# jan-frost/uzliti_slam

Hardware: AMD Instinct MI355X
Metric: SE(3) edges optimized/sec (node-pairs matched/sec in `secondary`) (higher is better)
Workload: dtype f64; 1 GPU; BASELINE config 2: 1000-node / 5000-edge SE(3) pose graph, 20 LM iterations, Huber(1) on loop closures; one independent graph per GPU; system_edges=4999

## Files before the change

uzliti_slam_amd/csrc/pgo_handle.hpp:

```cpp
#pragma once
#include "uzl_common.hpp"
#include "pgo_types.hpp"
#include "pgo_schur.hpp"
#include "pgo_ml_plan.hpp"
#include "pgo_lm.hpp"

#include <algorithm>
#include <chrono>
#include <cstdlib>
#include <cmath>
#include <functional>
#include <limits>
#include <new>
#include <numeric>

namespace uzl {
void k_prepare_nodes(const uzl_node* nodes, int n, int xy, double* pose, hipStream_t s);
void k_prepare_flat_nodes(const double* poses12, int n, double* pose, hipStream_t s);
void k_prepare_edges(const uzl_edge* edges, const int32_t* src, int e, const double* sensors, int ns, int xy, int odom_params,
                     double* zinv, double* info, hipStream_t s);
void k_prepare_flat_edges(const double* meas12, const double* info36, int e, double* zinv, double* info, hipStream_t s);
int k_chi2(const PgoDev& D, const double* pose, double delta, hipStream_t s);
int k_chi2_trial(const PgoDev& D, const double* pose, double delta, hipStream_t s);
hipError_t k_hessian(const PgoDev& D, const double* pose, double delta, int* g_edges, int* g_rows, hipStream_t s, bool with_chi2 = true, hipEvent_t ev_a = nullptr,
// ... 20 lines not shown
void k_poses_out(const double* pose, int n, double* out12, hipStream_t s);
void k_schur_gather(const PgoDev& D, const SchurDev& S, hipStream_t s);
void k_lm_head(const LmSlot* slots, int nslots, int pass_flags, hipStream_t s);
void k_lm_tail(const LmSlot* slots, int nslots, hipStream_t s);
hipError_t kl_linearize(const LmSlot* sl, int nslots, int g_edges, int g_asm, hipStream_t s);
void kl_eval(const LmSlot* sl, int nslots, int g_edges, int g_oplus, hipStream_t s);
void kl_schur_reduce(const LmSlot* sl, const LmShape& sh, hipStream_t s);
void kl_schur_backsub(const LmSlot* sl, const LmShape& sh, hipStream_t s);
void kl_schur_reduce(const HostSlot& hs, const LmShape& sh, hipStream_t s, KernelTimer* timer);
void kl_schur_backsub(const HostSlot& hs, const LmShape& sh, hipStream_t s, KernelTimer* timer);
void kl_ml_numeric(const LmSlot* sl, const LmShape& sh, int which, hipStream_t s);
void kl_ml_trial(const LmSlot* sl, const LmShape& sh, int which, int ns_steps, hipStream_t s);
void kl_ml_numeric(const HostSlot& hs, const LmShape& sh, hipStream_t s, KernelTimer* timer, const std::function<void()>& level1_done);
void kl_ml_trial(const HostSlot& hs, const LmShape& sh, int ns_steps, hipStream_t s, KernelTimer* timer);
void ml_cg_variant(const MlHot& ml, int agg, size_t lds_full, int32_t* variant, int32_t* comp_u, uint64_t* lds);
hipError_t kl_ml_init(const LmSlot* sl, const LmSlot* by_value, const LmShape& sh, hipStream_t s);
hipError_t kl_ml_pcg_its(const LmSlot* sl, const LmSlot* by_value, const LmShape& sh, int first, int n, hipStream_t s, hipEvent_t* ev = nullptr);
void kl_ml_pcg_init(const HostSlot& hs, const LmShape& sh, hipStream_t s);
void kl_ml_spmv(const HostSlot& hs, const LmShape& sh, int parity, hipStream_t s, hipEvent_t ev_a = nullptr, hipEvent_t ev_b = nullptr);
hipError_t kl_ml_cg(const HostSlot& hs, const LmShape& sh, int parity, int init, hipStream_t s, hipEvent_t ev_a = nullptr, hipEvent_t ev_b = nullptr);
}



namespace uzl { struct LmRun; }
using namespace uzl;

struct SysBufs {
    DevBuf<int32_t> row_ptr, col, rowhdr, b2v;
    DevBuf<double> blk, hdiag, minv, x, xs, r, z, p, p2, ap;
    std::vector<int32_t> upload(int nb, const std::vector<int32_t>& h_row_ptr, const std::vector<int32_t>& h_col, const std::vector<int32_t>& h_b2v, hipStream_t s)
    {
// ... 157 lines not shown
```

uzliti_slam_amd/csrc/pgo_lm.hpp:

```cpp
#pragma once
#include <cmath>
#include <hip/hip_runtime.h>

#include "pgo_types.hpp"

namespace uzl {

#define UZL_HD __host__ __device__ __forceinline__

constexpr double kResidualGuard = 0.25;
constexpr double kRateDrop = 0.6;
constexpr double kTolFloor2 = 1e-4;
constexpr double kStepT = 1.0, kStepR = 0.1;

UZL_HD double lm_cube(double t)
{
#pragma clang fp contract(off)
    const double p = t * t, pe = fma(t, t, -p);
    const double q = p * t, qe = fma(p, t, -q);
    return q + (qe + pe * t);
}

UZL_HD double lm_log(double x)
{
// ... 17 lines not shown
UZL_HD double lm_pcg_rate(double rz_stop, double rz_end, int its, double tol2, double tol_f2)
{
#pragma clang fp contract(off)
    const double rz0 = rz_stop / (tol2 * tol_f2);
    return (its >= 16 && rz0 > 0. && rz_end > 0. && rz_end < rz0) ? lm_log(rz0 / rz_end) / its : -1.;
}

UZL_HD bool lm_refresh(int it, int iterations, bool may_run_last, double last_rel, double refresh_rel, double rate_ref, double rate_last,
                       double rate_drop = kRateDrop)
{
#pragma clang fp contract(off)
    return it == 0 || ((last_rel > refresh_rel || (rate_ref > 0. && rate_last > 0. && rate_last < rate_drop * rate_ref)) &&
                       (may_run_last || it + 1 < iterations));
}

struct LmStep { double rho; bool accepted; double last_rel; };
UZL_HD LmStep lm_step(double current_chi, double temp_chi, double scale_sum, double& lambda, double& ni)
{
#pragma clang fp contract(off)
    LmStep r;
    const double scale = scale_sum + 1e-3;
    r.rho = (current_chi - temp_chi) / scale;
    r.accepted = r.rho > 0 && std::isfinite(temp_chi);
    r.last_rel = 0.;
    if (r.accepted) {
        double alpha = 1. - lm_cube(2 * r.rho - 1);
        alpha = alpha < 2. / 3. ? alpha : 2. / 3.;
        const double scaleFactor = (1. / 3. > alpha) ? 1. / 3. : alpha;
        lambda *= scaleFactor;
        ni = 2.;
// ... 11 lines not shown
```

uzliti_slam_amd/csrc/pgo_lm_kernels.hip:

```cpp
#include "pgo_device.hpp"
#include "pgo_lm.hpp"

namespace uzl {

__device__ __forceinline__ void lm_head_decide(const LmSlot& S, LmDev* lm, int phase, double chi, double dmax, int pass_flags)
{
    const int p = lm->pass + 1;
    lm->pass = p;
    double* __restrict__ scal = S.D.scal;
    int need = 0;
    if (phase == kLmLin) {
        scal[4] = chi; scal[6] = dmax;
        if (lm->it == 0) {
            lm->chi_cur = chi; lm->chi2_initial = chi;
            lm->lambda = 1e-5 * dmax;
            lm->ni = 2.;
        }
        lm->adopted = 0;
        if (lm->pending) { lm->ix ^= 1; lm->pending = 0; lm->adopted = 1; }
        if (lm_refresh(lm->it, lm->iterations, lm->sync_rebuild != 0, lm->last_rel, lm->refresh_rel, lm->rate_ref, lm->rate_last, lm->rate_drop)) {
            lm->st_precond_builds++;
            need |= (lm->it == 0 || lm->sync_rebuild) ? (kNeedNumeric | kNeedTrial) : kNeedRebuild;
        }
        lm->qmax = 0;
        if (S.red) lm->schur_pass = p;
    } else if (phase == kLmRetry) {
        if (S.red) lm->schur_pass = p;
    } else if (phase == kLmNeedSetup) {
        need = lm->need;
    } else {
        return;
    }
    const double lambda = lm->lambda;
    scal[3] = lambda; scal[8] = lm->tol_f2; scal[12] = lm->eps_t; scal[13] = lm->eps_r;
// ... 88 lines not shown
        ratio = bb > 0. ? rr / bb : 0.;
    }
    __shared__ uint32_t s_seq;
    if (tid == 0) {
        const uint32_t seq = (uint32_t)(lm->tails + 1);
        lm->tails = (int32_t)seq;
        s_seq = seq;
        double* __restrict__ scal = sscal;
        if (solving && !done) {
            if (lm->flags[1] >= lm->max_it) { lm->phase = kLmAnomaly; lm->anomaly_code = 1; lm->flags[0] = 1; }
        } else if (solving) {
            const int its = lm->flags[1];
            bool conv = lm->flags[2] == 0;
            if (conv) scal[7] = ratio;
            if (conv && lm->guarded && !(ratio <= kResidualGuard)) conv = false;
            if (!conv) { lm->phase = kLmAnomaly; lm->anomaly_code = lm->flags[2] ? 2 : 3; }
            else {
                scal[4] = chi_t; scal[5] = sc;
                lm->st_pcg_iterations += its; lm->st_lm_trials++; lm->pcg_last = its;
                const double rate = lm_pcg_rate(scal[1], scal[0], its, lm->tol2, lm->tol_f2);
                if (rate > 0.) { lm->rate_last = rate; if (lm->fresh || lm->rate_ref < 0.) lm->rate_ref = rate; }
                double lambda = lm->lambda, ni = lm->ni;
                const LmStep st = lm_step(lm->chi_cur, chi_t, sc, lambda, ni);
                lm->lambda = lambda; lm->ni = ni;
                if (st.accepted) { lm->last_rel = st.last_rel; lm->chi_cur = chi_t; lm->cur ^= 1; }
                const int qmax = lm->qmax + 1;
                lm->qmax = qmax;
                if (st.rho < 0 && qmax < 10) lm->phase = kLmRetry;
                else {
                    lm->st_iterations_done = lm->it + 1;
                    if (qmax == 10 || st.rho == 0) { lm->st_terminated_early = 1; lm->phase = kLmDone; }
// ... 34 lines not shown
```

uzliti_slam_amd/csrc/pgo_ml_kernels.hip:

```cpp
#include <hip/hip_ext.h>
#include <functional>
#include <mutex>
#include <type_traits>

#include "pgo_device.hpp"
#include "uzl_common.hpp"

namespace uzl {

#ifdef UZL_STAMPS
__device__ unsigned long long g_stamps[64];
#define STAMP_DECL unsigned long long st_prev_ = __builtin_amdgcn_s_memrealtime(); int st_i_ = 0;
#define STAMP(base) do { if (blockIdx.x == 0 && threadIdx.x == 0) { unsigned long long n_ = __builtin_amdgcn_s_memrealtime(); \
        atomicAdd(&g_stamps[(base) + st_i_], n_ - st_prev_); st_prev_ = n_; } st_i_++; } while (0)
#else
#define STAMP_DECL
#define STAMP(base) do { } while (0)
#endif

struct P3 { double X[9], Y[9], Z[9]; };

__device__ __forceinline__ void mat3(const double* A, const double* B, double* C)
{
#pragma unroll
// ... 1134 lines not shown
        sr1[tid] = s;
        if (gl == 1 && A1 < n1) rg[(size_t)A1 * 6 + k] = s;
    }
    __syncthreads();
    if (gl == 2 && tid < 6) {
        double s = 0.;
        for (int la = 0; la < kAggPerBlk; la++) {
            const int A1 = blockIdx.x * kAggPerBlk + la;
            if (A1 < n1) s += restrict_comp(H.geo[1] + (size_t)A1 * 3, sr1 + la * 6, tid);
        }
        rg[(size_t)blockIdx.x * 6 + tid] = s;
    }
    if (blockIdx.x == 0 && tid == 0) { D.flags[0] = 0; D.flags[1] = 0; D.flags[2] = 0; D.flags[3] = 0; D.scal[2] = 1.; }
}

__device__ __forceinline__ double dot6(double2 a0, double2 a1, double2 a2, double v0, double v1, double v2, double v3, double v4, double v5)
{
    double t = a0.x * v0;
    t = fma(a0.y, v1, t); t = fma(a1.x, v2, t); t = fma(a1.y, v3, t); t = fma(a2.x, v4, t); t = fma(a2.y, v5, t);
    return t;
}
template <int AGG>
__device__ __forceinline__ double sg_at(const double* __restrict__ Sg, int gl, int t)
{
    if (AGG == 1 || gl != 2) return Sg[t];
    const double2 v = reinterpret_cast<const double2*>(Sg)[t];
    return v.x + v.y;
}
constexpr int kSpmvWaves4 = 4;
__device__ __forceinline__ int xcd_contiguous(int b, int g)
{
    const int q = g >> 3, rem = g & 7, x = b & 7;
    return x * q + (x < rem ? x : rem) + (b >> 3);
}
template <int AGG, int RPW = AGG, int WAVES = (AGG == 1 ? 8 : kSpmvWaves4)>
__device__ __forceinline__ void ml_spmv_kernel_body(PgoDev D, MlHot H, const double* __restrict__ p_old,
                                                     double* __restrict__ p_new, int n_part, double tol2)
{
    constexpr int kWaves = WAVES, kRowsPerWave = RPW;
    constexpr bool kLds = (WAVES == 2);
    constexpr int kRowsPerBlk = kWaves * kRowsPerWave, kAggPerBlk = kRowsPerBlk / kMlFanout;
    constexpr int kGrpU = (kWaves >= 8) ? 2 : 4;
    __shared__ double sgrp[kMaxPartials / 64];
    __shared__ double slook[2][kMaxPartials / 64];
    constexpr int kGat = 2 + 3 * kRowsPerWave;
    __shared__ __attribute__((aligned(16))) double sgat[kWaves][kGat][64];
    __shared__ double sd[kRowsPerBlk * 6];
    __shared__ double sw[kRowsPerBlk * 6];
    __shared__ double ss1[kAggPerBlk * 6];
    __shared__ double sg1[kAggPerBlk * 3];
    const int done = D.flags[0];
    STAMP_DECL
    const int gl = (AGG == 1 || H.levels < 2) ? 1 : 2;
    const int tid = threadIdx.x, lane = tid & 63, wv = __builtin_amdgcn_readfirstlane(tid >> 6), g = lane / 6, r = lane % 6;
    const bool lact = lane < 60;
    const int bx = xcd_contiguous((int)blockIdx.x, (int)gridDim.x);
    const int row0 = bx * kRowsPerBlk + wv * kRowsPerWave;
    double vpart[kGrpU];
#pragma unroll
    for (int u = 0; u < kGrpU; u++) {
        const int i = (wv + u * kWaves) * 64 + lane;
        const double x = D.part_b[i < n_part ? i : 0];
        vpart[u] = (i < n_part) ? x : 0.;
    }
    double2 vlook[kGrpU];
    if (bx == 0) {
#pragma unroll
// ... 4 lines not shown
        }
    }
    const int it = D.flags[1];
    const double rz_prev = D.scal[2], thr_old = D.scal[1], lambda = D.scal[3], rz_last = D.scal[0];
    int s0[kRowsPerWave], s1[kRowsPerWave], cf[kRowsPerWave], cf2[kRowsPerWave];
#pragma unroll
    for (int q = 0; q < kRowsPerWave; q++) {
        const int a = row0 + q;
        const int32_t* __restrict__ hd = D.rowhdr + (size_t)(a < D.nb ? a : 0) * kRowHdr;
        s0[q] = (a < D.nb) ? hd[0] : 0;
        s1[q] = (a < D.nb) ? hd[1] : 0;
        cf[q] = (a < D.nb && lact) ? hd[2 + g] : -1;
        cf2[q] = (a < D.nb && lact) ? hd[12 + g] : -1;
    }
    if (done) return;
    double g1v = 0.;
    if (tid < kAggPerBlk * 3) {
        const int A1 = bx * kAggPerBlk + tid / 3;
        if (gl == 2 && A1 < H.n[1]) g1v = H.geo[1][(size_t)A1 * 3 + tid % 3];
    }
    const int gbase = g * 6;
    auto gather6 = [&](int slot, double v, int base, double& v0, double& v1, double& v2, double& v3, double& v4, double& v5) {
        double* line = sgat[wv][slot];
        line[lane] = v;
        __builtin_amdgcn_wave_barrier();
        const double2* __restrict__ p2 = reinterpret_cast<const double2*>(line + base);
        const double2 a = p2[0], b = p2[1], c = p2[2];
        v0 = a.x; v1 = a.y; v2 = b.x; v3 = b.y; v4 = c.x; v5 = c.y;
    };
    double hrow[6] = {0, 0, 0, 0, 0, 0}, zo_r = 0., po_r = 0.;
// ... 603 lines not shown
    const int done = D.flags[0];
    const int tid = threadIdx.x, t = blockIdx.x * 256 + tid, n6 = 6 * H.n[2];
    double vp[4];
    part_issue<256, 4>(D.part_a, n_part, tid, vp);
    double rgv = 0., sgv = 0.;
    if (t < n6) { rgv = rg_old[t]; sgv = sg_at<4>(H.Sg, 2, t); }
    const double rz = D.scal[0];
    if (done) return;
    const double pAp = block_sum_w<4>(part_fold<256, 4>(D.part_a, n_part, tid, vp), s4);
    const bool bad = !(pAp > 0.);
    const double alpha = bad ? 0. : rz / pAp;
    if (t < n6) H.Vg[t] = rgv - alpha * sgv;
    if (blockIdx.x == 0 && tid == 0) { D.scal[9] = alpha; D.scal[10] = bad ? 1. : 0.; }
}

template <int kCompU, bool kLds = false>
__device__ __forceinline__ void ml_cg_comp_kernel_body(PgoDev D, MlHot H, const double* __restrict__ p,
                                                           const double* __restrict__ rg_old, double* __restrict__ rg_new,
                                                           int n_part, int init)
{
    __shared__ double s3[3];
    __shared__ double sv[kCgBlk];
    __shared__ double sw[kCgBlk];
    __shared__ double sy[6];
    __shared__ double szj[48];
    __shared__ double scomp[3][6];
    __shared__ double spm[6];
    if (D.flags[0]) return;
    const int tid = threadIdx.x;
    const int a = blockIdx.x * kMlFanout + tid / 6, r = tid % 6;
    const bool act = tid < 48 && a < D.nb;
    const int n1 = H.n[1], ng6 = 6 * n1;
    double vpart[4] = {0., 0., 0., 0.};
    if (!init) part_issue<kCgBlk, 4>(D.part_a, n_part, tid, vpart);
    double xv = 0., xsv = 0., rv0 = 0., apv = 0., pv = 0., geo[12] = {0, 0, 0, 0, 0, 0, 0, 0, 0, 0, 0, 0};
    const int look = init ? 1 : D.flags[3];
    const double unit = progress_unit(D.scal, r);
    if (act) {
        const size_t i = (size_t)a * 6 + r;
        rv0 = D.r[i];
        if (!init) { xv = D.x[i]; xsv = D.xs[i]; apv = D.ap[i]; pv = p[i]; }
        const double* __restrict__ gg = H.geo0 + (size_t)a * 12;
#pragma unroll
// ... 7 lines not shown
        for (int c = 0; c < 6; c++) { const double2 v = src[c]; w0[2 * c] = v.x; w0[2 * c + 1] = v.y; }
    }
    const double rz = init ? 0. : D.scal[0];
    double rgreg[kCompU], sgreg[kCompU];
    float cm[6][kCompU];
    const int cst = H.c32_stride;
    const float* __restrict__ crow = H.Cmat32 + (size_t)blockIdx.x * 6 * cst;
#pragma unroll
    for (int u = 0; u < kCompU; u++) {
        const int t = u * kCgBlk + tid;
        const bool in = t < ng6;
        rgreg[u] = in ? rg_old[t] : 0.;
        sgreg[u] = (!init && in) ? H.Sg[t] : 0.;
#pragma unroll
        for (int q = 0; q < 6; q++) { const float y = crow[(size_t)q * cst + (in ? t : 0)]; cm[q][u] = in ? y : 0.f; }
    }
    double alpha = 0.;
    bool bad = false;
    if (!init) {
        const double pAp = block_sum_w<3, kLds>(part_fold<kCgBlk, 4>(D.part_a, n_part, tid, vpart), s3);
        bad = !(pAp > 0.);
        alpha = bad ? 0. : rz / pAp;
    }
    {
        double ps[6] = {0, 0, 0, 0, 0, 0};
#pragma unroll
        for (int u = 0; u < kCompU; u++) {
            const double v = fma(-alpha, sgreg[u], rgreg[u]);
#pragma unroll
            for (int q = 0; q < 6; q++) ps[q] = fma((double)cm[q][u], v, ps[q]);
// ... 297 lines not shown
    const auto* lm = state_of(S, slots);
    const int ix = lm->ix;
    if (init) {
        if (!init_due(lm)) return;
        ml_cg_kernel_body<AGG, COMP, YPRE, false>(S.Dp, hot_of(S, ix), S.pbuf[0], rg_of(S, ix, 0), rg_of(S, ix, 1), 0, 1);
    } else ml_cg_kernel_body<AGG, COMP, YPRE, VPRE>(S.Dp, hot_of(S, ix), S.pbuf[parity ^ 1], rg_of(S, ix, parity ^ 1), rg_of(S, ix, parity), S.g_spmv, 0);
}
template <class SLOT>
__global__ __launch_bounds__(256) void ml_alpha_lm_kernel(const SLOT slots, int parity)
{
    const LmSlot& S = slot_of(slots);
    const auto* lm = state_of(S, slots);
    ml_alpha_kernel_body(S.Dp, hot_of(S, lm->ix), rg_of(S, lm->ix, parity ^ 1), S.g_spmv);
}

static hipError_t lm_cg_lds(const void* fn, int variant_ix, size_t lds)
{
    constexpr int kMaxDev = 16, kVar = 24;
    static size_t configured_tab[kMaxDev][kVar] = {};
    static std::mutex mu;
    int dev = 0;
    if (hipGetDevice(&dev) != hipSuccess || dev < 0 || dev >= kMaxDev) dev = 0;
    std::lock_guard<std::mutex> lock(mu);
    if (lds > configured_tab[dev][variant_ix]) {
        const hipError_t e = hipFuncSetAttribute(fn, hipFuncAttributeMaxDynamicSharedMemorySize, (int)lds);
        if (e != hipSuccess) return e;
        configured_tab[dev][variant_ix] = lds;
    }
    return hipSuccess;
}

template <class SLOT>
static hipError_t kl_ml_cg_t(SLOT sl, const LmShape& sh, int parity, int init, hipStream_t s, hipEvent_t ev_a = nullptr, hipEvent_t ev_b = nullptr)
{
    constexpr int kSlotKind = std::is_pointer<SLOT>::value ? 0 : (std::is_same<SLOT, LmSlot>::value ? 1 : 2);
    const dim3 g(sh.g_rows, 1, sh.nslots), t(kCgBlk);
    const size_t lds = (size_t)sh.cg_lds;
    if (lds > kMlLdsLimit) return hipErrorInvalidValue;
    auto cg = [&](auto kernel) {
        const hipError_t e = lm_cg_lds(reinterpret_cast<const void*>(kernel), 8 * kSlotKind + sh.cg_variant, lds);
        if (e == hipSuccess) launch(kernel, g, t, lds, s, ev_a, ev_b, sl, parity, init);
        return e;
    };
    switch (sh.cg_variant) {
    case kCgComp1: {
        const int u = sh.comp_u;
        auto kernel = sh.batch_geometry ? (u <= 5 ? ml_cg_comp_lm_kernel<5, true, SLOT> : ml_cg_comp_lm_kernel<8, true, SLOT>)
                    : u <= 5 ? ml_cg_comp_lm_kernel<5, false, SLOT> : u <= 8 ? ml_cg_comp_lm_kernel<8, false, SLOT>
                    : u <= 12 ? ml_cg_comp_lm_kernel<12, false, SLOT> : ml_cg_comp_lm_kernel<16, false, SLOT>;
        launch(kernel, g, t, 0, s, ev_a, ev_b, sl, parity, init);
        return hipSuccess; }
    case kCgPlain1: return cg(ml_cg_lm_kernel<1, false, false, false, SLOT>);
    case kCgPlain4: return cg(ml_cg_lm_kernel<4, false, false, false, SLOT>);
    case kCgComp4: return cg(ml_cg_lm_kernel<4, true, false, false, SLOT>);
    case kCgComp4Ypre: return cg(ml_cg_lm_kernel<4, true, true, false, SLOT>);
    case kCgComp4Vpre:
        if (!init) hipLaunchKernelGGL((ml_alpha_lm_kernel<SLOT>), dim3((6 * sh.n_lv[2] + 255) / 256, 1, sh.nslots), dim3(256), 0, s, sl, parity);
        return cg(ml_cg_lm_kernel<4, true, false, true, SLOT>);
    }
    return hipErrorInvalidValue;
// ... 20 lines not shown
void ml_cg_variant(const MlHot& ml, int agg, size_t lds_full, int32_t* variant, int32_t* comp_u, uint64_t* lds)
{
    *comp_u = 0; *lds = lds_full;
    if (agg == 1) {
        if (!ml.Cmat) { *variant = kCgPlain1; return; }
        const int cols = 6 * ml.n[1];
        *variant = kCgComp1; *lds = 0;
        *comp_u = cols <= 5 * kCgBlk ? 5 : (cols <= 8 * kCgBlk ? 8 : (cols <= 12 * kCgBlk ? 12 : 16));
        return;
    }
    if (!ml.Cmat) { *variant = kCgPlain4; return; }
    *lds = ml_comp4_lds(ml.n[2]);
    const bool ypre = ml.levels >= 2 && 6 * ml.n[2] <= 4 * 32 * kYU;
    *variant = ypre ? kCgComp4Ypre : (ml.Vg != nullptr ? kCgComp4Vpre : kCgComp4);
}
hipError_t kl_ml_init(const LmSlot* sl, const LmSlot* by_value, const LmShape& sh, hipStream_t s)
{
    if (by_value && sh.nslots == 1) { kl_ml_init_t<LmSlot>(*by_value, sh, s); return kl_ml_cg_t<LmSlot>(*by_value, sh, 0, 1, s); }
    kl_ml_init_t<const LmSlot*>(sl, sh, s);
    return kl_ml_cg_t<const LmSlot*>(sl, sh, 0, 1, s);
}
hipError_t kl_ml_pcg_its(const LmSlot* sl, const LmSlot* by_value, const LmShape& sh, int first, int n, hipStream_t s, hipEvent_t* ev)
{
    const bool one = by_value && sh.nslots == 1 && !ev;
    for (int q = 0; q < n; q++) {
        const int par = (first + q) & 1;
        hipError_t e;
        if (ev) { kl_ml_spmv_t<const LmSlot*>(sl, sh, par, s, ev[4 * q], ev[4 * q + 1]); e = kl_ml_cg_t<const LmSlot*>(sl, sh, par, 0, s, ev[4 * q + 2], ev[4 * q + 3]); }
        else if (one) { kl_ml_spmv_t<LmSlot>(*by_value, sh, par, s); e = kl_ml_cg_t<LmSlot>(*by_value, sh, par, 0, s); }
        else { kl_ml_spmv_t<const LmSlot*>(sl, sh, par, s); e = kl_ml_cg_t<const LmSlot*>(sl, sh, par, 0, s); }
        if (e != hipSuccess) return e;
    }
    return hipSuccess;
}
void kl_ml_pcg_init(const HostSlot& hs, const LmShape& sh, hipStream_t s) { kl_ml_init_t<HostSlot>(hs, sh, s); }
void kl_ml_spmv(const HostSlot& hs, const LmShape& sh, int parity, hipStream_t s, hipEvent_t ev_a, hipEvent_t ev_b) { kl_ml_spmv_t<HostSlot>(hs, sh, parity, s, ev_a, ev_b); }
hipError_t kl_ml_cg(const HostSlot& hs, const LmShape& sh, int parity, int init, hipStream_t s, hipEvent_t ev_a, hipEvent_t ev_b)
{
    return kl_ml_cg_t<HostSlot>(hs, sh, parity, init, s, ev_a, ev_b);
}

}

#ifdef UZL_STAMPS
extern "C" UZL_DIAG_EXPORT int uzl_debug_read_stamps(unsigned long long* out, int reset)
{
    if (hipMemcpyFromSymbol(out, HIP_SYMBOL(uzl::g_stamps), sizeof(unsigned long long) * 64) != hipSuccess) return -3;
    if (reset) { unsigned long long z[64] = {0}; if (hipMemcpyToSymbol(HIP_SYMBOL(uzl::g_stamps), z, sizeof(z)) != hipSuccess) return -3; }
    return 0;
}
#endif

#ifdef UZL_DIAG
// ... 51 lines not shown
```

uzliti_slam_amd/csrc/pgo_types.hpp:

```cpp
#pragma once
#include <cstdint>
#include "../../include/uzl_mi355x.h"

namespace uzl {
constexpr size_t kMlLdsLimit = (size_t)140 * 1024;
__host__ __device__ inline size_t ml_comp4_lds(int n2) { return (size_t)6 * (size_t)n2 * 8 + 64; }


constexpr int kMaxPartials = 8192;
constexpr int kProgressEvery = 2;
constexpr int kRowHdr = 24;

struct PgoDev {
    int32_t n, nb, e, nslots;
    int32_t e_begin, e_end;
    int32_t diag_owner;
    int32_t sibling0;
    double* pose;
    double* pose_trial;
    const int32_t* v2b;
    const int32_t* b2v;
    const int32_t* ei;
    const int32_t* ej;
    const double* zinv;
// ... 157 lines not shown
    double* rg[2][2];
    double* dense[2][kMlMaxLevels + 1];
    double* nsT[2];
    double* nsX[2];
    double* pbuf[2];
    double* pose[2];
    int32_t g_edges, g_asm, g_oplus, g_rows, g_spmv, red, pad0, pad1;
    int64_t copy_stride;
};
struct HostSlot {
    LmSlot S;
    int32_t ix, cur;
    double tol2;
};

enum LmCgVariant : int32_t { kCgPlain1 = 0, kCgComp1 = 1, kCgPlain4 = 2, kCgComp4 = 3, kCgComp4Ypre = 4, kCgComp4Vpre = 5 };
struct LmShape {
    int32_t nslots;
    int32_t batch_geometry;
    int32_t levels, cl, agg;
    int32_t mult, ns_steps, upper_ns;
    int32_t cg_variant, comp_u;
    int32_t n_lv[kMlMaxLevels + 2];
    int32_t work_t[kMlMaxLevels + 2];
    int32_t chunks[kMlMaxLevels + 2];
    int32_t inner_aggs;
    int32_t g_edges, g_asm, g_oplus, g_rows, g_spmv;
    int32_t red, schur_runs, schur_backsub_grid;
    int64_t schur_items;
    uint64_t cg_lds;
// ... 11 lines not shown
```

uzliti_slam_amd/csrc/uzl_pgo_lm.hip:

```cpp
#include "pgo_handle.hpp"

namespace uzl {

struct LmRun {
    int nslots = 0;
    DevBuf<LmSlot> d_slots;
    DevBuf<LmDev> d_lm;
    PinBuf<LmHost> h_pub;
    LmHost* d_pub = nullptr;
    PinBuf<LmDev> h_init;
    std::vector<LmSlot> slots;
    LmShape shape{};
    DevBuf<double> d_start;
    hipEvent_t ev_fork = nullptr, ev_join = nullptr;
    bool join_pending = false;
    uint64_t gen = ~0ull;
    int solves_of_gen = 0;
    int first_solve_its = 0;
    std::vector<std::vector<int>> trial_its_prev, trial_its_cur;
    std::vector<uint64_t> hist_gen;
    struct Seg { hipGraph_t g = nullptr; hipGraphExec_t x = nullptr; };
    Seg setup, reb, pcg_long;
    void drop(Seg& q) { if (q.x) { (void)hipGraphExecDestroy(q.x); q.x = nullptr; } if (q.g) { (void)hipGraphDestroy(q.g); q.g = nullptr; } }
    void drop_all() { drop(setup); drop(reb); drop(pcg_long); }
};

void lm_run_destroy(LmRun* r)
{
    if (!r) return;
    r->drop_all();
    if (r->ev_fork) (void)hipEventDestroy(r->ev_fork);
    if (r->ev_join) (void)hipEventDestroy(r->ev_join);
    delete r;
}

namespace {

LmRun* new_run()
{
// ... 20 lines not shown
    UZL_HIP(kl_linearize(R->d_slots.p, sh.nslots, sh.g_edges, sh.g_asm, s));
}
void enq_head(LmRun* R, int pass_flags, bool linearized, hipStream_t s)
{
    const LmShape& sh = R->shape;
    if (!linearized) enq_linearize(R, s);
    k_lm_head(R->d_slots.p, sh.nslots, pass_flags, s);
    if (sh.red) kl_schur_reduce(R->d_slots.p, sh, s);
}
void enq_setup(LmRun* R, int which, int ns_steps, hipStream_t s)
{
    kl_ml_numeric(R->d_slots.p, R->shape, which, s);
    kl_ml_trial(R->d_slots.p, R->shape, which, ns_steps, s);
}
const LmSlot* by_value_slot(LmRun* R) { return (R->shape.nslots == 1 && !R->shape.batch_geometry) ? R->slots.data() : nullptr; }
void enq_init(LmRun* R, hipStream_t s) { UZL_HIP(kl_ml_init(R->d_slots.p, by_value_slot(R), R->shape, s)); }
void enq_pcg(LmRun* R, int first, int n, hipStream_t s, hipEvent_t* ev = nullptr) { UZL_HIP(kl_ml_pcg_its(R->d_slots.p, by_value_slot(R), R->shape, first, n, s, ev)); }
void enq_tail(LmRun* R, hipStream_t s)
{
    const LmShape& sh = R->shape;
    if (sh.red) kl_schur_backsub(R->d_slots.p, sh, s);
    kl_eval(R->d_slots.p, sh.nslots, sh.g_edges, sh.g_oplus, s);
    k_lm_tail(R->d_slots.p, sh.nslots, s);
}
template <class F>
void run_seg(LmRun::Seg& q, bool eager, hipStream_t s, F&& enqueue)
{
    if (eager) { enqueue(s); return; }
    if (!q.x) {
        UZL_HIP(hipStreamBeginCapture(s, hipStreamCaptureModeThreadLocal));
        try { enqueue(s); }
        catch (...) {
// ... 220 lines not shown
                }
                const bool no_history = jobs[(size_t)slot_job[sl]].h->cfg.pass_history == 1;
                auto up = [&](int count) { return nS == 1 ? count + 1 : ((count + 2) & ~1); };
                w = v.pcg_last > 0 ? up(v.pcg_last) : ((R->first_solve_its > 0 && !no_history) ? up(R->first_solve_its) : 2 * kLong);
                if (v.pcg_last > 0 && prev_last[sl] > 0 && v.pcg_last > prev_last[sl]) w = up(v.pcg_last + std::min(v.pcg_last - prev_last[sl], 16));
                {
                    const std::vector<int>& hist = R->trial_its_prev[(size_t)slot_job[sl]];
                    if (!no_history && (size_t)v.st_lm_trials < hist.size()) w = std::max(w, up(hist[(size_t)v.st_lm_trials]));
                }
                w = std::min(w, ((v.max_it + 1) & ~1));
            }
            want = std::max(want, w);
        }
        want = std::max(2, want);
        const int base = (nS == 1 && slot_job[0] >= 0 && snap[0].lm.phase == kLmSolve) ? snap[0].lm.flags[1] : 0;
        mark(0);
        if (any_start && R->join_pending) { UZL_HIP(hipStreamWaitEvent(s, R->ev_join, 0)); R->join_pending = false; }
        mark(1);
        if (any_start) enq_head(R, pf, lin_ahead, s);
        lin_ahead = false;
        mark(2);
        if (pf & kPassSetup) {
            const int steps = nS == 1 ? ml_ns_steps_at(R->shape.ns_steps, snap[0].lm.it) : R->shape.ns_steps;
            if (steps != R->shape.ns_steps) enq_setup(R, 1, steps, s);
            else run_seg(R->setup, eager, s, [&](hipStream_t q) { enq_setup(R, 1, steps, q); });
        }
        if (pf & kPassRebuild) {
            UZL_HIP(hipEventRecord(R->ev_fork, s));
            UZL_HIP(hipStreamWaitEvent(o.s2, R->ev_fork, 0));
            run_seg(R->reb, eager, o.s2, [&](hipStream_t q) { enq_setup(R, 0, R->shape.ns_steps, q); });
            UZL_HIP(hipEventRecord(R->ev_join, o.s2));
            R->join_pending = true;
        }
        mark(3);
        if (any_start) enq_init(R, s);
        mark(4);
        if (o.timer && o.timer->on) {
            std::vector<hipEvent_t> ev((size_t)4 * want);
            for (int q = 0; q < want; q++) { o.timer->pair(o.spmv_name, &ev[4 * q], &ev[4 * q + 1]); o.timer->pair(o.cg_name, &ev[4 * q + 2], &ev[4 * q + 3]); }
            enq_pcg(R, base, want, s, ev.data());
        } else {
            int first = base, left = want;
            if (!eager && (first & 1)) { enq_pcg(R, first, 1, s); first++; left--; }
            const int n_long = eager ? 0 : left / kLong, rem = left - n_long * kLong;
            for (int i = 0; i < n_long; i++) run_seg(R->pcg_long, false, s, [&](hipStream_t q) { enq_pcg(R, 0, kLong, q); });
            if (rem > 0) enq_pcg(R, first + n_long * kLong, rem, s);
        }
        mark(5);
        enq_tail(R, s);
        if (!R->join_pending && !(o.timer && o.timer->on)) { enq_linearize(R, s); lin_ahead = true; }
        mark(6);
        passes++;
        for (int sl = 0; sl < nS; sl++) sent[sl]++;
        const auto tp1 = std::chrono::steady_clock::now();
        if (o.verbose) fprintf(stderr, "[uzl_pgo]   pass %d enqueued: segments %d, %d PCG iterations, %d graph(s) in the slots\n", passes - 1, pf, want, n_active);
        bool refill = false;
        for (int sl = 0; sl < nS; sl++) {
            if (slot_job[sl] < 0 || jobs[slot_job[sl]].finished) continue;
            (void)wait_pub(s, R, sl, sent[sl], &snap[sl]);
            LmJob& J = jobs[slot_job[sl]];
            const LmDev& v = snap[sl].lm;
// ... 164 lines not shown
```

Measured before the change: 17.23 million edges/s.

## Pass compact PCG kernel arguments with host-resolved buffer index

Adds a compact PcgArgs struct (at most 256 bytes) for single-slot PCG kernels. The host resolves the double-buffer index and tolerance ahead of time and bakes them into the kernel arguments, so kernels no longer dereference the LmSlot through device memory to find their buffers. Each captured PCG graph segment is now kept per buffer index. The device still checks that its LM index matches the one the host predicted and raises a new breakdown anomaly code if they disagree. This adds complexity and a risk that the host-side index prediction goes wrong.

```diff
diff --git a/uzliti_slam_amd/csrc/pgo_handle.hpp b/uzliti_slam_amd/csrc/pgo_handle.hpp
--- a/uzliti_slam_amd/csrc/pgo_handle.hpp
+++ b/uzliti_slam_amd/csrc/pgo_handle.hpp
@@ -58,8 +58,8 @@
 void kl_ml_numeric(const HostSlot& hs, const LmShape& sh, hipStream_t s, KernelTimer* timer, const std::function<void()>& level1_done);
 void kl_ml_trial(const HostSlot& hs, const LmShape& sh, int ns_steps, hipStream_t s, KernelTimer* timer);
 void ml_cg_variant(const MlHot& ml, int agg, size_t lds_full, int32_t* variant, int32_t* comp_u, uint64_t* lds);
-hipError_t kl_ml_init(const LmSlot* sl, const LmSlot* by_value, const LmShape& sh, hipStream_t s);
-hipError_t kl_ml_pcg_its(const LmSlot* sl, const LmSlot* by_value, const LmShape& sh, int first, int n, hipStream_t s, hipEvent_t* ev = nullptr);
+hipError_t kl_ml_init(const LmSlot* sl, const LmSlot* by_value, const LmShape& sh, int ix, hipStream_t s);
+hipError_t kl_ml_pcg_its(const LmSlot* sl, const LmSlot* by_value, const LmShape& sh, int ix, double tol2, int first, int n, hipStream_t s, hipEvent_t* ev = nullptr);
 void kl_ml_pcg_init(const HostSlot& hs, const LmShape& sh, hipStream_t s);
 void kl_ml_spmv(const HostSlot& hs, const LmShape& sh, int parity, hipStream_t s, hipEvent_t ev_a = nullptr, hipEvent_t ev_b = nullptr);
 hipError_t kl_ml_cg(const HostSlot& hs, const LmShape& sh, int parity, int init, hipStream_t s, hipEvent_t ev_a = nullptr, hipEvent_t ev_b = nullptr);
diff --git a/uzliti_slam_amd/csrc/pgo_lm.hpp b/uzliti_slam_amd/csrc/pgo_lm.hpp
--- a/uzliti_slam_amd/csrc/pgo_lm.hpp
+++ b/uzliti_slam_amd/csrc/pgo_lm.hpp
@@ -55,6 +55,8 @@
                        (may_run_last || it + 1 < iterations));
 }
 
+UZL_HD int lm_pass_ix(int phase, int ix, int pending) { return (phase == kLmLin && pending) ? (ix ^ 1) : ix; }
+
 struct LmStep { double rho; bool accepted; double last_rel; };
 UZL_HD LmStep lm_step(double current_chi, double temp_chi, double scale_sum, double& lambda, double& ni)
 {
diff --git a/uzliti_slam_amd/csrc/pgo_lm_kernels.hip b/uzliti_slam_amd/csrc/pgo_lm_kernels.hip
--- a/uzliti_slam_amd/csrc/pgo_lm_kernels.hip
+++ b/uzliti_slam_amd/csrc/pgo_lm_kernels.hip
@@ -16,8 +16,9 @@
             lm->lambda = 1e-5 * dmax;
             lm->ni = 2.;
         }
-        lm->adopted = 0;
-        if (lm->pending) { lm->ix ^= 1; lm->pending = 0; lm->adopted = 1; }
+        lm->adopted = lm->pending ? 1 : 0;
+        lm->ix = lm_pass_ix(phase, lm->ix, lm->pending);
+        lm->pending = 0;
         if (lm_refresh(lm->it, lm->iterations, lm->sync_rebuild != 0, lm->last_rel, lm->refresh_rel, lm->rate_ref, lm->rate_last, lm->rate_drop)) {
             lm->st_precond_builds++;
             need |= (lm->it == 0 || lm->sync_rebuild) ? (kNeedNumeric | kNeedTrial) : kNeedRebuild;
@@ -136,7 +137,7 @@
             bool conv = lm->flags[2] == 0;
             if (conv) scal[7] = ratio;
             if (conv && lm->guarded && !(ratio <= kResidualGuard)) conv = false;
-            if (!conv) { lm->phase = kLmAnomaly; lm->anomaly_code = lm->flags[2] ? 2 : 3; }
+            if (!conv) { lm->phase = kLmAnomaly; lm->anomaly_code = lm->flags[2] == kBreakdownIx ? 4 : (lm->flags[2] ? 2 : 3); }
             else {
                 scal[4] = chi_t; scal[5] = sc;
                 lm->st_pcg_iterations += its; lm->st_lm_trials++; lm->pcg_last = its;
diff --git a/uzliti_slam_amd/csrc/pgo_ml_kernels.hip b/uzliti_slam_amd/csrc/pgo_ml_kernels.hip
--- a/uzliti_slam_amd/csrc/pgo_ml_kernels.hip
+++ b/uzliti_slam_amd/csrc/pgo_ml_kernels.hip
@@ -1172,6 +1172,11 @@
     if (blockIdx.x == 0 && tid == 0) { D.flags[0] = 0; D.flags[1] = 0; D.flags[2] = 0; D.flags[3] = 0; D.scal[2] = 1.; }
 }
 
+__device__ __forceinline__ void pcg_ix_mismatch(int32_t* flags)
+{
+    if (blockIdx.x == 0 && threadIdx.x == 0) { flags[0] = 1; flags[2] = kBreakdownIx; }
+}
+
 __device__ __forceinline__ double dot6(double2 a0, double2 a1, double2 a2, double v0, double v1, double v2, double v3, double v4, double v5)
 {
     double t = a0.x * v0;
@@ -1193,7 +1198,8 @@
 }
 template <int AGG, int RPW = AGG, int WAVES = (AGG == 1 ? 8 : kSpmvWaves4)>
 __device__ __forceinline__ void ml_spmv_kernel_body(PgoDev D, MlHot H, const double* __restrict__ p_old,
-                                                     double* __restrict__ p_new, int n_part, double tol2)
+                                                     double* __restrict__ p_new, int n_part, double tol2,
+                                                     const int32_t* ix_word = nullptr, int ix = 0, bool ix_check = false)
 {
     constexpr int kWaves = WAVES, kRowsPerWave = RPW;
     constexpr bool kLds = (WAVES == 2);
@@ -1209,6 +1215,7 @@
     __shared__ double sg1[kAggPerBlk * 3];
     const int done = D.flags[0];
     STAMP_DECL
+    const int ix_dev = ix_word ? *ix_word : 0;
     const int gl = (AGG == 1 || H.levels < 2) ? 1 : 2;
     const int tid = threadIdx.x, lane = tid & 63, wv = __builtin_amdgcn_readfirstlane(tid >> 6), g = lane / 6, r = lane % 6;
     const bool lact = lane < 60;
@@ -1243,6 +1250,7 @@
         cf2[q] = (a < D.nb && lact) ? hd[12 + g] : -1;
     }
     if (done) return;
+    if (ix_check && ix_dev != ix) { pcg_ix_mismatch(D.flags); return; }
     double g1v = 0.;
     if (tid < kAggPerBlk * 3) {
         const int A1 = bx * kAggPerBlk + tid / 3;
@@ -1876,10 +1884,11 @@
     if (blockIdx.x == 0 && tid == 0) { D.scal[9] = alpha; D.scal[10] = bad ? 1. : 0.; }
 }
 
-template <int kCompU, bool kLds = false>
+template <int kCompU, bool kLds = false, bool kLate = false>
 __device__ __forceinline__ void ml_cg_comp_kernel_body(PgoDev D, MlHot H, const double* __restrict__ p,
                                                            const double* __restrict__ rg_old, double* __restrict__ rg_new,
-                                                           int n_part, int init)
+                                                           int n_part, int init, const int32_t* ix_word = nullptr, int ix = 0,
+                                                           bool ix_check = false, const LmDev* lm = nullptr)
 {
     __shared__ double s3[3];
     __shared__ double sv[kCgBlk];
@@ -1888,7 +1897,12 @@
     __shared__ double szj[48];
     __shared__ double scomp[3][6];
     __shared__ double spm[6];
-    if (D.flags[0]) return;
+    STAMP_DECL
+    if (!kLate && D.flags[0]) return;
+    const int done = kLate ? D.flags[0] : 0;
+    const int ix_dev = kLate ? *ix_word : 0;
+    int ph = kLmSolve, ip = 0, ps = 0;
+    if (kLate && lm && init) { ph = lm->phase; ip = lm->init_pass; ps = lm->pass; }
     const int tid = threadIdx.x;
     const int a = blockIdx.x * kMlFanout + tid / 6, r = tid % 6;
     const bool act = tid < 48 && a < D.nb;
@@ -1926,6 +1940,14 @@
         sgreg[u] = (!init && in) ? H.Sg[t] : 0.;
 #pragma unroll
         for (int q = 0; q < 6; q++) { const float y = crow[(size_t)q * cst + (in ? t : 0)]; cm[q][u] = in ? y : 0.f; }
+    }
+    STAMP(32);
+#ifdef UZL_STAMPS
+    if (blockIdx.x == 0 && tid == 0) atomicAdd(&g_stamps[46], 1ull);
+#endif
+    if (kLate) {
+        if (ix_check && ix_dev != ix) { pcg_ix_mismatch(D.flags); return; }
+        if (done || !(ph == kLmSolve && ip == ps)) return;
     }
     double alpha = 0.;
     bool bad = false;
@@ -2253,6 +2275,62 @@
     ml_alpha_kernel_body(S.Dp, hot_of(S, lm->ix), rg_of(S, lm->ix, parity ^ 1), S.g_spmv);
 }
 
+__device__ __forceinline__ PgoDev pcg_dev(const PcgArgs& A)
+{
+    PgoDev D = {};
+    D.nb = A.nb; D.diag_owner = A.diag_owner;
+    D.col = A.col; D.rowhdr = A.rowhdr; D.blk = A.blk; D.hdiag = A.hdiag;
+    D.b = A.b; D.x = A.x; D.xs = A.xs; D.r = A.r; D.z = A.z; D.ap = A.ap;
+    D.part_a = A.part_a; D.part_b = A.part_b; D.part_c = A.part_c; D.scal = A.scal; D.flags = A.flags;
+    return D;
+}
+__device__ __forceinline__ MlHot pcg_hot(const PcgArgs& A)
+{
+    MlHot H = {};
+    H.levels = 1; H.n[1] = A.n1;
+    H.geo0 = A.geo0; H.Winv[0] = A.Winv0; H.Cmat32 = A.Cmat32; H.c32_stride = A.c32_stride; H.Sg = A.Sg;
+    return H;
+}
+__global__ __launch_bounds__(kCgBlk) void ml_init_pcg_kernel(const PcgArgs A)
+{
+    if (A.lm) {
+        if (A.lm->ix != A.ix) { pcg_ix_mismatch(A.flags); return; }
+        if (!init_due(A.lm)) return;
+    }
+    ml_init_kernel_body<1>(pcg_dev(A), pcg_hot(A), A.pbuf[0], A.pbuf[1], A.rg[0]);
+}
+__global__ __launch_bounds__(512) __attribute__((amdgpu_waves_per_eu(4))) void ml_spmv_pcg_kernel(const PcgArgs A, int parity)
+{
+    double* const p0 = A.pbuf[0]; double* const p1 = A.pbuf[1];
+    int zero;
+    asm("s_mov_b32 %0, 0 ; ml_spmv: arguments fetched" : "=s"(zero)
+        : "s"(A.flags), "s"(A.lm), "s"(A.scal), "s"(A.part_b), "s"(A.rowhdr), "s"(A.part_a), "s"(A.part_c), "s"(A.hdiag),
+          "s"(A.z), "s"(A.blk), "s"(p0), "s"(p1), "s"(A.ap), "s"(A.geo0), "s"(A.Sg), "s"(A.col), "s"(__double_as_longlong(A.tol2)),
+          "s"(A.nb), "s"(A.n1), "s"(A.diag_owner), "s"(A.g_rows), "s"(A.ix), "s"(parity), "s"((int)gridDim.x));
+    PgoDev D = pcg_dev(A);
+    D.flags += zero; D.scal += zero; D.part_b += zero; D.part_c += zero; D.rowhdr += zero;
+    const int32_t* ix_word = (A.lm ? &A.lm->ix : A.flags) + zero;
+    ml_spmv_kernel_body<1, 1, 8>(D, pcg_hot(A), parity ? p1 : p0, parity ? p0 : p1, A.g_rows, A.tol2, ix_word, A.ix, A.lm != nullptr);
+}
+template <int kCompU, bool kInit>
+__global__ __launch_bounds__(kCgBlk) void ml_cg_comp_pcg_kernel(const PcgArgs A, int parity)
+{
+    constexpr int init = kInit ? 1 : 0;
+    double* const p0 = A.pbuf[0]; double* const p1 = A.pbuf[1];
+    double* const r0 = A.rg[0]; double* const r1 = A.rg[1];
+    int zero;
+    asm("s_mov_b32 %0, 0 ; ml_cg_comp: arguments fetched" : "=s"(zero)
+        : "s"(A.flags), "s"(A.lm), "s"(A.scal), "s"(A.part_a), "s"(A.r), "s"(A.part_b), "s"(A.part_c), "s"(A.z), "s"(p0), "s"(p1),
+          "s"(A.x), "s"(A.xs), "s"(A.ap), "s"(A.geo0), "s"(A.Winv0), "s"(A.Cmat32), "s"(r0), "s"(r1), "s"(A.Sg),
+          "s"(A.nb), "s"(A.n1), "s"(A.c32_stride), "s"(A.g_spmv), "s"(A.ix), "s"(parity));
+    PgoDev D = pcg_dev(A);
+    D.flags += zero; D.scal += zero; D.part_a += zero; D.r += zero;
+    const int32_t* ix_word = (A.lm ? &A.lm->ix : A.flags) + zero;
+    const bool odd = init || parity;
+    ml_cg_comp_kernel_body<kCompU, false, true>(D, pcg_hot(A), odd ? p0 : p1, odd ? r0 : r1, odd ? r1 : r0, init ? 0 : A.g_spmv, init,
+                                                ix_word, A.ix, A.lm != nullptr, A.lm);
+}
+
 static hipError_t lm_cg_lds(const void* fn, int variant_ix, size_t lds)
 {
     constexpr int kMaxDev = 16, kVar = 24;
@@ -2282,7 +2360,9 @@
         return e;
     };
     switch (sh.cg_variant) {
-    case kCgComp1: {
+    case kCgComp1:
+        if constexpr (!std::is_pointer<SLOT>::value) return hipErrorInvalidValue;
+        else {
         const int u = sh.comp_u;
         auto kernel = sh.batch_geometry ? (u <= 5 ? ml_cg_comp_lm_kernel<5, true, SLOT> : ml_cg_comp_lm_kernel<8, true, SLOT>)
                     : u <= 5 ? ml_cg_comp_lm_kernel<5, false, SLOT> : u <= 8 ? ml_cg_comp_lm_kernel<8, false, SLOT>
@@ -2333,29 +2413,77 @@
     const bool ypre = ml.levels >= 2 && 6 * ml.n[2] <= 4 * 32 * kYU;
     *variant = ypre ? kCgComp4Ypre : (ml.Vg != nullptr ? kCgComp4Vpre : kCgComp4);
 }
-hipError_t kl_ml_init(const LmSlot* sl, const LmSlot* by_value, const LmShape& sh, hipStream_t s)
-{
+static bool pcg_args_shape(const LmShape& sh) { return sh.nslots == 1 && !sh.batch_geometry && sh.agg == 1 && sh.cg_variant == kCgComp1; }
+static PcgArgs make_pcg_args(const LmSlot& S, const LmDev* lm, int ix, double tol2)
+{
+    const int64_t off = ix ? S.copy_stride : 0;
+    auto at = [off](auto* q) { return q ? reinterpret_cast<decltype(q)>(reinterpret_cast<uintptr_t>(q) + (uintptr_t)off) : q; };
+    const PgoDev& D = S.Dp;
+    const MlHot& H = S.hot[0];
+    PcgArgs A;
+    memset(&A, 0, sizeof(A));
+    A.flags = D.flags; A.scal = D.scal; A.part_a = D.part_a; A.part_b = D.part_b; A.part_c = D.part_c;
+    A.rowhdr = D.rowhdr; A.hdiag = D.hdiag; A.z = D.z; A.blk = D.blk; A.pbuf[0] = S.pbuf[0]; A.pbuf[1] = S.pbuf[1];
+    A.r = D.r; A.x = D.x; A.xs = D.xs; A.ap = D.ap;
+    A.geo0 = at(H.geo0); A.Winv0 = at(H.Winv[0]); A.Cmat32 = at(H.Cmat32); A.rg[0] = at(S.rg[0][0]); A.rg[1] = at(S.rg[0][1]);
+    A.Sg = H.Sg; A.lm = lm; A.col = D.col; A.b = D.b; A.tol2 = tol2;
+    A.nb = D.nb; A.n1 = H.n[1]; A.c32_stride = H.c32_stride; A.diag_owner = D.diag_owner;
+    A.g_rows = S.g_rows; A.g_spmv = S.g_spmv; A.ix = ix;
+    return A;
+}
+static void pcg_init(const PcgArgs& A, hipStream_t s) { hipLaunchKernelGGL(ml_init_pcg_kernel, dim3(A.g_rows), dim3(kCgBlk), 0, s, A); }
+static void pcg_spmv(const PcgArgs& A, int parity, hipStream_t s, hipEvent_t ev_a = nullptr, hipEvent_t ev_b = nullptr)
+{
+    launch(ml_spmv_pcg_kernel, dim3(A.g_spmv), dim3(512), 0, s, ev_a, ev_b, A, parity);
+}
+static void pcg_cg(const PcgArgs& A, int comp_u, int parity, int init, hipStream_t s, hipEvent_t ev_a = nullptr, hipEvent_t ev_b = nullptr)
+{
+    auto pick = [&](auto k5, auto k8, auto k12, auto k16) { return comp_u <= 5 ? k5 : comp_u <= 8 ? k8 : comp_u <= 12 ? k12 : k16; };
+    auto kernel = init ? pick(ml_cg_comp_pcg_kernel<5, true>, ml_cg_comp_pcg_kernel<8, true>, ml_cg_comp_pcg_kernel<12, true>, ml_cg_comp_pcg_kernel<16, true>)
+                       : pick(ml_cg_comp_pcg_kernel<5, false>, ml_cg_comp_pcg_kernel<8, false>, ml_cg_comp_pcg_kernel<12, false>, ml_cg_comp_pcg_kernel<16, false>);
+    launch(kernel, dim3(A.g_rows), dim3(kCgBlk), 0, s, ev_a, ev_b, A, parity);
+}
+
+hipError_t kl_ml_init(const LmSlot* sl, const LmSlot* by_value, const LmShape& sh, int ix, hipStream_t s)
+{
+    if (by_value && pcg_args_shape(sh)) {
+        const PcgArgs A = make_pcg_args(*by_value, by_value->lm, ix, 0.);
+        pcg_init(A, s); pcg_cg(A, sh.comp_u, 0, 1, s);
+        return hipSuccess;
+    }
     if (by_value && sh.nslots == 1) { kl_ml_init_t<LmSlot>(*by_value, sh, s); return kl_ml_cg_t<LmSlot>(*by_value, sh, 0, 1, s); }
     kl_ml_init_t<const LmSlot*>(sl, sh, s);
     return kl_ml_cg_t<const LmSlot*>(sl, sh, 0, 1, s);
 }
-hipError_t kl_ml_pcg_its(const LmSlot* sl, const LmSlot* by_value, const LmShape& sh, int first, int n, hipStream_t s, hipEvent_t* ev)
+hipError_t kl_ml_pcg_its(const LmSlot* sl, const LmSlot* by_value, const LmShape& sh, int ix, double tol2, int first, int n, hipStream_t s, hipEvent_t* ev)
 {
     const bool one = by_value && sh.nslots == 1 && !ev;
+    const bool args = one && pcg_args_shape(sh);
+    const PcgArgs A = args ? make_pcg_args(*by_value, by_value->lm, ix, tol2) : PcgArgs{};
     for (int q = 0; q < n; q++) {
         const int par = (first + q) & 1;
         hipError_t e;
-        if (ev) { kl_ml_spmv_t<const LmSlot*>(sl, sh, par, s, ev[4 * q], ev[4 * q + 1]); e = kl_ml_cg_t<const LmSlot*>(sl, sh, par, 0, s, ev[4 * q + 2], ev[4 * q + 3]); }
+        if (args) { pcg_spmv(A, par, s); pcg_cg(A, sh.comp_u, par, 0, s); e = hipSuccess; }
+        else if (ev) { kl_ml_spmv_t<const LmSlot*>(sl, sh, par, s, ev[4 * q], ev[4 * q + 1]); e = kl_ml_cg_t<const LmSlot*>(sl, sh, par, 0, s, ev[4 * q + 2], ev[4 * q + 3]); }
         else if (one) { kl_ml_spmv_t<LmSlot>(*by_value, sh, par, s); e = kl_ml_cg_t<LmSlot>(*by_value, sh, par, 0, s); }
         else { kl_ml_spmv_t<const LmSlot*>(sl, sh, par, s); e = kl_ml_cg_t<const LmSlot*>(sl, sh, par, 0, s); }
         if (e != hipSuccess) return e;
     }
     return hipSuccess;
 }
-void kl_ml_pcg_init(const HostSlot& hs, const LmShape& sh, hipStream_t s) { kl_ml_init_t<HostSlot>(hs, sh, s); }
-void kl_ml_spmv(const HostSlot& hs, const LmShape& sh, int parity, hipStream_t s, hipEvent_t ev_a, hipEvent_t ev_b) { kl_ml_spmv_t<HostSlot>(hs, sh, parity, s, ev_a, ev_b); }
+void kl_ml_pcg_init(const HostSlot& hs, const LmShape& sh, hipStream_t s)
+{
+    if (pcg_args_shape(sh)) pcg_init(make_pcg_args(hs.S, nullptr, hs.ix, hs.tol2), s);
+    else kl_ml_init_t<HostSlot>(hs, sh, s);
+}
+void kl_ml_spmv(const HostSlot& hs, const LmShape& sh, int parity, hipStream_t s, hipEvent_t ev_a, hipEvent_t ev_b)
+{
+    if (pcg_args_shape(sh)) pcg_spmv(make_pcg_args(hs.S, nullptr, hs.ix, hs.tol2), parity, s, ev_a, ev_b);
+    else kl_ml_spmv_t<HostSlot>(hs, sh, parity, s, ev_a, ev_b);
+}
 hipError_t kl_ml_cg(const HostSlot& hs, const LmShape& sh, int parity, int init, hipStream_t s, hipEvent_t ev_a, hipEvent_t ev_b)
 {
+    if (pcg_args_shape(sh)) { pcg_cg(make_pcg_args(hs.S, nullptr, hs.ix, hs.tol2), sh.comp_u, parity, init, s, ev_a, ev_b); return hipSuccess; }
     return kl_ml_cg_t<HostSlot>(hs, sh, parity, init, s, ev_a, ev_b);
 }
 
diff --git a/uzliti_slam_amd/csrc/pgo_types.hpp b/uzliti_slam_amd/csrc/pgo_types.hpp
--- a/uzliti_slam_amd/csrc/pgo_types.hpp
+++ b/uzliti_slam_amd/csrc/pgo_types.hpp
@@ -195,6 +195,36 @@
     double tol2;
 };
 
+constexpr int32_t kBreakdownIx = 2;
+struct PcgArgs {
+    int32_t* flags;
+    double* scal;
+    double* part_a;
+    double* part_b;
+    double* part_c;
+    const int32_t* rowhdr;
+    double* hdiag;
+    double* z;
+    double* blk;
+    double* pbuf[2];
+    double* r;
+    double* x;
+    double* xs;
+    double* ap;
+    const double* geo0;
+    const double* Winv0;
+    const float* Cmat32;
+    double* rg[2];
+    double* Sg;
+    const LmDev* lm;
+    const int32_t* col;
+    double* b;
+    double tol2;
+    int32_t nb, n1, c32_stride, diag_owner;
+    int32_t g_rows, g_spmv, ix, pad0;
+};
+static_assert(sizeof(PcgArgs) <= 256, "PcgArgs: four cache lines of kernel-argument memory");
+
 enum LmCgVariant : int32_t { kCgPlain1 = 0, kCgComp1 = 1, kCgPlain4 = 2, kCgComp4 = 3, kCgComp4Ypre = 4, kCgComp4Vpre = 5 };
 struct LmShape {
     int32_t nslots;
diff --git a/uzliti_slam_amd/csrc/uzl_pgo_lm.hip b/uzliti_slam_amd/csrc/uzl_pgo_lm.hip
--- a/uzliti_slam_amd/csrc/uzl_pgo_lm.hip
+++ b/uzliti_slam_amd/csrc/uzl_pgo_lm.hip
@@ -20,9 +20,9 @@
     std::vector<std::vector<int>> trial_its_prev, trial_its_cur;
     std::vector<uint64_t> hist_gen;
     struct Seg { hipGraph_t g = nullptr; hipGraphExec_t x = nullptr; };
-    Seg setup, reb, pcg_long;
+    Seg setup, reb, pcg_long[2];
     void drop(Seg& q) { if (q.x) { (void)hipGraphExecDestroy(q.x); q.x = nullptr; } if (q.g) { (void)hipGraphDestroy(q.g); q.g = nullptr; } }
-    void drop_all() { drop(setup); drop(reb); drop(pcg_long); }
+    void drop_all() { drop(setup); drop(reb); drop(pcg_long[0]); drop(pcg_long[1]); }
 };
 
 void lm_run_destroy(LmRun* r)
@@ -73,8 +73,11 @@
     kl_ml_trial(R->d_slots.p, R->shape, which, ns_steps, s);
 }
 const LmSlot* by_value_slot(LmRun* R) { return (R->shape.nslots == 1 && !R->shape.batch_geometry) ? R->slots.data() : nullptr; }
-void enq_init(LmRun* R, hipStream_t s) { UZL_HIP(kl_ml_init(R->d_slots.p, by_value_slot(R), R->shape, s)); }
-void enq_pcg(LmRun* R, int first, int n, hipStream_t s, hipEvent_t* ev = nullptr) { UZL_HIP(kl_ml_pcg_its(R->d_slots.p, by_value_slot(R), R->shape, first, n, s, ev)); }
+void enq_init(LmRun* R, int ix, hipStream_t s) { UZL_HIP(kl_ml_init(R->d_slots.p, by_value_slot(R), R->shape, ix, s)); }
+void enq_pcg(LmRun* R, int ix, double tol2, int first, int n, hipStream_t s, hipEvent_t* ev = nullptr)
+{
+    UZL_HIP(kl_ml_pcg_its(R->d_slots.p, by_value_slot(R), R->shape, ix, tol2, first, n, s, ev));
+}
 void enq_tail(LmRun* R, hipStream_t s)
 {
     const LmShape& sh = R->shape;
@@ -325,6 +328,9 @@
         }
         want = std::max(2, want);
         const int base = (nS == 1 && slot_job[0] >= 0 && snap[0].lm.phase == kLmSolve) ? snap[0].lm.flags[1] : 0;
+        static const bool wrong_ix = diag_flag("UZL_LM_WRONG_IX");
+        const int pass_ix = lm_pass_ix(snap[0].lm.phase, snap[0].lm.ix, snap[0].lm.pending) ^ (wrong_ix ? 1 : 0);
+        const double tol2 = snap[0].lm.tol2;
         mark(0);
         if (any_start && R->join_pending) { UZL_HIP(hipStreamWaitEvent(s, R->ev_join, 0)); R->join_pending = false; }
         mark(1);
@@ -344,18 +350,18 @@
             R->join_pending = true;
         }
         mark(3);
-        if (any_start) enq_init(R, s);
+        if (any_start) enq_init(R, pass_ix, s);
         mark(4);
         if (o.timer && o.timer->on) {
             std::vector<hipEvent_t> ev((size_t)4 * want);
             for (int q = 0; q < want; q++) { o.timer->pair(o.spmv_name, &ev[4 * q], &ev[4 * q + 1]); o.timer->pair(o.cg_name, &ev[4 * q + 2], &ev[4 * q + 3]); }
-            enq_pcg(R, base, want, s, ev.data());
+            enq_pcg(R, pass_ix, tol2, base, want, s, ev.data());
         } else {
             int first = base, left = want;
-            if (!eager && (first & 1)) { enq_pcg(R, first, 1, s); first++; left--; }
+            if (!eager && (first & 1)) { enq_pcg(R, pass_ix, tol2, first, 1, s); first++; left--; }
             const int n_long = eager ? 0 : left / kLong, rem = left - n_long * kLong;
-            for (int i = 0; i < n_long; i++) run_seg(R->pcg_long, false, s, [&](hipStream_t q) { enq_pcg(R, 0, kLong, q); });
-            if (rem > 0) enq_pcg(R, first + n_long * kLong, rem, s);
+            for (int i = 0; i < n_long; i++) run_seg(R->pcg_long[pass_ix], false, s, [&](hipStream_t q) { enq_pcg(R, pass_ix, tol2, 0, kLong, q); });
+            if (rem > 0) enq_pcg(R, pass_ix, tol2, first + n_long * kLong, rem, s);
         }
         mark(5);
         enq_tail(R, s);
```

Result: faster. 18.75 million edges/s (median of 6 runs) (+8.8%).
